# xguo7/SND-VAE

Measured on AMD Instinct MI355X. Metric: training graphs/sec + ELBO-step ms, N=4096 d=64, at 1/2/4/8 MI355X, higher is better.
Workload: dtype bf16; 1 GPU; C2: node-latent SND-VAE train step, N=4096, d=64, 8 graphs/GPU, HIP-graph replay; n_nodes=4096, latent=64, graphs_per_gpu=8, global_batch=8, parallelism=dp1, hip_graph=True

## Files before the change

### snd_vae_amd/csrc/snd_common.hpp

```cpp
#pragma once
#include <hip/hip_runtime.h>
#include <cstdint>
#include <cstdio>
#include <string>

#include "../../include/snd_vae.h"

namespace snd {

void set_error(const char* fmt, ...);

#define SND_CHECK_ARG(cond, ...)                                   \
  do {                                                             \
    if (!(cond)) {                                                 \
      ::snd::set_error(__VA_ARGS__);                               \
      return SND_ERR_ARG;                                          \
    }                                                              \
  } while (0)

#define SND_LAUNCH_CHECK(what)                                     \
  do {                                                             \
    hipError_t e_ = hipGetLastError();                             \
    if (e_ != hipSuccess) {                                        \
      ::snd::set_error("%s: %s", what, hipGetErrorString(e_));     \
      return SND_ERR_HIP;                                          \
    }                                                              \
  } while (0)

#define SND_TRY(expr)                                              \
  do {                                                             \
    int rc_ = (expr);                                              \
    if (rc_ != 0) return rc_;                                      \
  } while (0)

constexpr float kBnC = 0.99950037468777325f;
constexpr float kLeak = 0.2f;
constexpr float kLog2e = 1.4426950408889634f;
constexpr float kLn2 = 0.69314718055994531f;
constexpr double kSoftplusM1 = 0.31326168751822286;

#ifndef SND_MEAS
#define SND_MEAS 0
#endif
constexpr int kKeepDbg = 1 << 23;
__host__ __device__ __forceinline__ constexpr int kdbg(int dbg) { return SND_MEAS ? dbg : (dbg & kKeepDbg); }

__device__ __forceinline__ float lrelu(float x) { return fmaxf(x, kLeak * x); }
__device__ __forceinline__ float lrelu_grad(float x) { return x >= 0.f ? 1.f : kLeak; }

inline int device_cu_count() {
  static const int n = [] {
    int d = 0, v = 0;
    if (hipGetDevice(&d) != hipSuccess ||
        hipDeviceGetAttribute(&v, hipDeviceAttributeMultiprocessorCount, d) != hipSuccess || v <= 0) {
      (void)hipGetLastError();
      return 256;
    }
    return v;
  }();
  return n;
}

__device__ __forceinline__ void edge_ce_terms(float x, float pw, float& coef, float& loss) {
  coef = -pw;
  if (pw != 1.f) {
    const float e = __expf(-fabsf(x));
    const float q = 1.f + e;
    const float r = __builtin_amdgcn_rcpf(q);
    const float sg = x >= 0.f ? r : e * r;
    coef += (pw - 1.f) * sg;
    loss += (pw - 1.f) * (fmaxf(x, 0.f) + __logf(q));
  }
}

__device__ __forceinline__ float kl_elem(float s, float mu) {
  const float x = 2.f * s;
  float r;
// ... 113 lines not shown
```

### snd_vae_amd/csrc/snd_dec.hip

```cpp
#include "snd_dec.hpp"

#include <algorithm>

namespace snd {
namespace {

constexpr int DT = 1024;
constexpr int NW = DT / 64;
constexpr int kDynLds = 148 * 1024;

typedef __attribute__((address_space(1))) const void* gptr_t;
typedef __attribute__((address_space(3))) void* lptr_t;

__device__ __forceinline__ void dglds16(const void* g, void* lds_base) {
  __builtin_amdgcn_global_load_lds((gptr_t)g, (lptr_t)lds_base, 16, 0, 0);
}
__host__ __device__ __forceinline__ int dswz(int row, int kp) {
  return kp == 128 ? (row & 15) : (kp == 64 ? ((row >> 1) & 7) : 0);
}
__host__ __device__ __forceinline__ int lkc_of(int kp) { return kp == 128 ? 4 : (kp == 64 ? 3 : 2); }
__host__ __device__ __forceinline__ int img_bytes(int rows, int kp) {
  return ((rows * kp * 2) + 1023) & ~1023;
}
__host__ __device__ __forceinline__ int rup(int a, int b) { return (a + b - 1) / b * b; }
// ... 21 lines not shown
    ldY2n = rup(max(p.m2.b, 1), 4);
    w = 0; a = wb; b = a + max(ja, ua); c = b + max(u1, u3);
    total = c + TR * ldY2n * 4;
  }
};
struct BwdLay {
  int w, d3, d2, d1, cps, total, tapb;
  __host__ __device__ BwdLay(const DecChainBwdArgs& p, int TR, bool str = false) {
    tapb = max(max(tap_bytes(p.k3t), tap_bytes(p.k2t)), tap_bytes(p.k1t));
    const int wb = str ? 2 * tapb : max(max(p.k3t.np * p.k3t.kp, p.k2t.np * p.k2t.kp), p.k1t.np * p.k1t.kp) * 5 * 2;
    const int nw = NW;
    w = 0;
    d3 = wb;
    d2 = d3 + img_bytes(in_rows(TR + 8), p.k3t.kp);
    d1 = d2 + img_bytes(in_rows(TR + 4), p.k2t.kp);
    cps = d1 + img_bytes(in_rows(TR), p.k1t.kp);
    const int c1 = (nw / ((p.k2t.np / 16 + 1) / 2)) * 3 * p.k2t.np;
    const int c2 = (nw / (p.k3t.np / 16)) * 3 * p.k3t.np;
    total = cps + max(c1, c2) * 4;
  }
};

struct Tile { int r0, rend, glo, ghi; };
template <int TR>
__device__ __forceinline__ Tile tile_of(int t, int npg) {
  const int tpg = (npg + TR - 1) / TR;
  const int g = t / tpg, lt = t - g * tpg;
  Tile x;
  x.glo = g * npg; x.ghi = x.glo + npg;
  x.r0 = x.glo + lt * TR; x.rend = min(x.r0 + TR, x.ghi);
  return x;
}

template <int NWV = NW>
__device__ __forceinline__ void stage_window(const __bf16* src, int ld, int K, int wr0, int nrows,
                                             int nvalid, int glo, int ghi, int kp, char* img,
                                             const void* zero) {
  const int lane = threadIdx.x & 63, w = threadIdx.x >> 6;
  const int lk = lkc_of(kp), kc = 1 << lk;
  const int npc = ((nrows << lk) + 63) >> 6;
  for (int j = w; j < npc; j += NWV) {
    const int q = (j << 6) + lane;
    const int row = q >> lk, pc = q & (kc - 1);
    const int c = pc ^ dswz(row, kp);
    const int gr = wr0 + row;
    const bool v = row < nvalid && gr >= glo && gr < ghi && 8 * c < K;
    const void* g = v ? (const void*)(src + (long long)gr * ld + 8 * c) : zero;
    dglds16(g, img + (j << 10));
  }
}
__device__ __forceinline__ void stage_weights(const DecImg& im, char* dst, int dbg) {
  if (dbg & 1) return;
  const int lane = threadIdx.x & 63, w = threadIdx.x >> 6;
  const int npc = (5 * im.np * im.kp * 2) >> 10;
  const char* g = reinterpret_cast<const char*>(im.w) + lane * 16;
  for (int j = w; j < npc; j += NW) dglds16(g + (j << 10), dst + (j << 10));
}
__device__ __forceinline__ void dglds16_async(const void* g, void* lds_base) {
  const unsigned dst = __builtin_amdgcn_readfirstlane((unsigned)(uintptr_t)(lptr_t)lds_base);
  unsigned keep;
  asm volatile("s_mov_b32 %0, m0\n\ts_mov_b32 m0, %2\n\ts_nop 0\n\t"
               "global_load_lds_dwordx4 %1, off\n\ts_mov_b32 m0, %0"
               : "=&s"(keep) : "v"(g), "s"(dst) : "memory");
}
__device__ __forceinline__ void stage_weights_async(const DecImg& im, char* dst, int dbg) {
  if (dbg & 1) return;
  const int lane = threadIdx.x & 63, w = threadIdx.x >> 6;
  const int npc = (5 * im.np * im.kp * 2) >> 10;
  const char* g = reinterpret_cast<const char*>(im.w) + lane * 16;
  for (int j = w; j < npc; j += NW) dglds16_async(g + (j << 10), dst + (j << 10));
}
template <int NWV>
__device__ __forceinline__ void stage_tap_async(const DecImg& im, int t, char* dst, int dbg) {
  if (dbg & 1) return;
  const int lane = threadIdx.x & 63, w = threadIdx.x >> 6;
  const int npc = tap_bytes(im) >> 10;
  const char* g = reinterpret_cast<const char*>(im.w) + (long long)t * tap_bytes(im) + lane * 16;
  for (int j = w; j < npc; j += NWV) dglds16_async(g + (j << 10), dst + (j << 10));
}
__host__ __device__ __forceinline__ int wimg_bytes(const DecImg& im) { return 5 * im.np * im.kp * 2; }
__device__ __forceinline__ void wait_dma() {
  __builtin_amdgcn_s_waitcnt(0x0F70);
  __syncthreads();
}

__device__ __forceinline__ __bf16* img_at(__bf16* img, int row, int kp, int n0) {
  return img + row * kp + ((((n0 >> 3) ^ dswz(row, kp)) << 3) | (n0 & 4));
}

template <int NBH, int KCS, class Pre, class Epi>
__device__ __forceinline__ void conv_phase_t(const __bf16* xs, int kpx, const __bf16* ws, int kpw, int np,
                                             int n_out, Pre&& pre, Epi&& epi, int dbg) {
  const int lane = threadIdx.x & 63, w = __builtin_amdgcn_readfirstlane(threadIdx.x >> 6);
  const int li = lane & 15, lg = lane >> 4;
  const int nrb = (n_out + 15) >> 4, nbc = np >> 4;
  const int ncg = (nbc + NBH - 1) / NBH, wpc = NW / ncg;
// ... 93 lines not shown
        const __bf16* xrp = xs + xrow * kpx;
        const int xsw = dswz(xrow, kpx);
        auto chunk = [&](int ks) {
          const int ch = 4 * ks + lg;
          const bf16x8 bx = *reinterpret_cast<const bf16x8*>(xrp + ((ch ^ xsw) << 3));
#pragma unroll
          for (int i = 0; i < NBH; ++i) {
            const bf16x8 aw = *reinterpret_cast<const bf16x8*>(wrp + wb[i] + ((ch ^ wsw) << 3));
            acc[j][i] = __builtin_amdgcn_mfma_f32_16x16x32_bf16(aw, bx, acc[j][i], 0, 0, 0);
          }
        };
        if (KCS > 0 && kpw == 32 * KCS) {
#pragma unroll
          for (int ks = 0; ks < KCS; ++ks) chunk(ks);
        } else {
          for (int ks = 0; ks < (kpw >> 5); ++ks) chunk(ks);
        }
      }
    }
  }
  if (!act) return;
#pragma unroll
  for (int j = 0; j < MAXRB; ++j) {
    const int rb = k0 + j * wpc;
    if (rb >= nrb) break;
    epi(16 * rb + li, nb0, acc[j], yp[j]);
  }
}

__device__ __forceinline__ float colpar(const ColMap& m, int n, const float* A, const float* Bv) {
  if (!m.valid(n) || !A) return 0.f;
  if (n < m.a || !Bv) return A[n < m.a ? n : m.logical(n)];
  return Bv[n - m.offb];
}

template <int CIN, int COUT, int SCR>
__device__ __forceinline__ void head_tile(int hi, int orow, bool rv, long long gr, const float (&u)[CIN],
                                          const float (&yv)[CIN], const float* hp, const float (&tg)[COUT],
                                          float count, float* yhat, __bf16* dyp, float* scr,
                                          double* sscr) {
  float wv[CIN][COUT], bv[COUT], gk[CIN], bk[CIN];
#pragma unroll
  for (int k = 0; k < CIN; ++k) {
#pragma unroll
    for (int o = 0; o < COUT; ++o) wv[k][o] = hp[k * COUT + o];
    gk[k] = hp[24 + k] * kBnC;
    bk[k] = hp[24 + CIN + k];
  }
#pragma unroll
  for (int o = 0; o < COUT; ++o) bv[o] = hp[20 + o];
  float dp[COUT];
  double sse = 0.0;
#pragma unroll
  for (int o = 0; o < COUT; ++o) {
    float zo = bv[o];
#pragma unroll
    for (int k = 0; k < CIN; ++k) zo += u[k] * wv[k][o];
    const float yh = 1.f / (1.f + __expf(-zo));
    const float diff = yh - tg[o];
    if (rv) {
      if (yhat) yhat[gr * COUT + o] = yh;
      sse += (double)diff * diff;
    }
    dp[o] = rv ? 2.f * diff / count * yh * (1.f - yh) : 0.f;
  }
  float dt[CIN], dyv[CIN];
// ... 49 lines not shown
  __bf16* u2img = jimg;
  __bf16* u1img = reinterpret_cast<__bf16*>(smem + L.b);
  float* u3 = reinterpret_cast<float*>(smem + L.b);
  float* y3 = u3 + TR * 16;
  float* y2n = reinterpret_cast<float*>(smem + L.c);
  const int kpu2 = a.m2.phys() <= 32 ? 32 : (a.m2.phys() <= 64 ? 64 : 128);
  const int own = tl.rend - tl.r0;
  const bool stamp = kdbg(a.dbg) & (1 << 21);
  unsigned long long ts[9] = {};
  if (stamp) ts[0] = __builtin_amdgcn_s_memrealtime();

  if (kdbg(a.dbg) & (1 << 23)) {
    for (int i = tid * 16; i < L.total - L.a; i += DTK * 16)
      *reinterpret_cast<uint4*>(smem + L.a + i) = make_uint4(~0u, ~0u, ~0u, ~0u);
    __syncthreads();
  }
  if (!(kdbg(a.dbg) & 32)) {
    const int kpo = a.k2.kp, npc = (kpo - a.k1.np) >> 2, nr = in_rows(TR + 4);
    for (int i = tid; i < nr * 4; i += DTK) {
      const int row = i >> 2, q = i & 3;
      if (q < npc) *reinterpret_cast<bf16x4*>(img_at(u1img, row, kpo, a.k1.np + 4 * q)) = bf16x4{};
    }
  }
  __syncthreads();
  if (!(kdbg(a.dbg) & 16))
    stage_window<NWV>(a.zb, a.ldz, a.dj, tl.r0 - 6, in_rows(TR + 8), own + 12, tl.glo, tl.ghi, a.k1.kp,
                      reinterpret_cast<char*>(jimg), a.zero);
  char* tb0 = reinterpret_cast<char*>(wimg);
  char* tb1 = tb0 + L.tapb;
  if constexpr (STR) stage_tap_async<NWV>(a.k1, 0, tb0, kdbg(a.dbg));
  else stage_weights(a.k1, reinterpret_cast<char*>(wimg), kdbg(a.dbg));
  constexpr int HPT = DTK == 1024 ? 512 : DTK - 128;
  static_assert(DTK - 128 >= 2 * TR || DTK == 1024, "dec_fwd: head parameter threads overlap the targets'");
  if (tid >= HPT && tid < HPT + 128) {
    const int i = tid - HPT, hh = i >> 6, j = i & 63;
    const int cin = hh ? 20 : 10, cout = hh ? 1 : 2;
    const float* w = hh ? a.wn : a.ws;
    const float* b = hh ? a.bn : a.bs;
    const float* g = hh ? a.g2n : a.g3;
    const float* be = hh ? a.be2n : a.be3;
    float v = 0.f;
    if (j < cin * cout) v = w[j];
    else if (j >= 20 && j < 20 + cout) v = b[j - 20];
    else if (j >= 24 && j < 24 + cin) v = g[j - 24];
    else if (j >= 24 + cin && j < 24 + 2 * cin) v = be[j - 24 - cin];
    hp[hh][j] = v;
  }
  float tg[2] = {0.f, 0.f};
  if (tid < 2 * TR) {
    const int orow = tid % TR;
    const long long gr = tl.r0 + orow;
    if (orow < own) {
      if (tid < TR) { tg[0] = a.s_truth[gr * 2]; tg[1] = a.s_truth[gr * 2 + 1]; }
      else tg[0] = a.x_truth[gr];
    }
  }
  if (tid < 128) {
    const int n = tid;
    cp1[0][n] = colpar(a.m1, n, a.b1, nullptr);
    cp1[1][n] = colpar(a.m1, n, a.g1, nullptr) * kBnC;
    cp1[2][n] = colpar(a.m1, n, a.be1, nullptr);
    cp2[0][n] = colpar(a.m2, n, a.b2s, a.b2n);
    cp2[1][n] = colpar(a.m2, n, a.g2s, a.g2n) * kBnC;
    cp2[2][n] = colpar(a.m2, n, a.be2s, a.be2n);
    if (n < 16) {
      const ColMap m3{a.s3, 0, a.s3};
      cp3[0][n] = colpar(m3, n, a.b3, nullptr);
      cp3[1][n] = colpar(m3, n, a.g3, nullptr) * kBnC;
      cp3[2][n] = colpar(m3, n, a.be3, nullptr);
    }
  }
  wait_dma();
  if (stamp) ts[1] = __builtin_amdgcn_s_memrealtime();

  auto nopre = [](int, int, auto&) {};
  {
    const int wr0 = tl.r0 - 4, n_out = own + 8, kpo = a.k2.kp, nbc = a.k1.np >> 4;
    auto epi1 = [&](int orow, int nb0, f32x4 (&acc)[2], f32x4 (&)[2]) {
      if (orow >= n_out) return;
      const int gr = wr0 + orow;
      const bool ing = gr >= tl.glo && gr < tl.ghi, mine = gr >= tl.r0 && gr < tl.rend;
#pragma unroll
      for (int i = 0; i < 2; ++i) {
        if (nb0 + i >= nbc) continue;
        const int n0 = 16 * (nb0 + i) + 4 * lg;
        const f32x4 b = *reinterpret_cast<const f32x4*>(&cp1[0][n0]);
        const f32x4 g = *reinterpret_cast<const f32x4*>(&cp1[1][n0]);
        const f32x4 be = *reinterpret_cast<const f32x4*>(&cp1[2][n0]);
        f32x4 yv;
        bf16x4 ub;
#pragma unroll
        for (int e = 0; e < 4; ++e) {
          yv[e] = acc[i][e] + b[e];
          ub[e] = (__bf16)(ing ? lrelu(yv[e] * g[e] + be[e]) : 0.f);
        }
        *reinterpret_cast<bf16x4*>(img_at(u1img, orow, kpo, n0)) = ub;
        if (mine && !(kdbg(a.dbg) & 8)) {
          *reinterpret_cast<f32x4*>(a.y1 + (long long)gr * a.ldy1 + n0) = yv;
          *reinterpret_cast<bf16x4*>(a.u1 + (long long)gr * a.ldy1 + n0) = ub;
        }
      }
    };
// ... 97 lines not shown
        }
        const float t1[1] = {tg[0]};
        head_tile<20, 1, SCR>(1, orow, rv, gr, u, yv, hp[1], t1, a.cnt_n, a.xhat, a.dy2 + gr * a.lddy2 + a.m2.offb,
                              scr + NQS * SCR, sscr + TR);
      }
    }
    __syncthreads();
    if (stamp) ts[7] = __builtin_amdgcn_s_memrealtime();
    if (tid < NQS + NQN) {
      const float* src = scr + tid * SCR;
      float v = 0.f;
#pragma unroll 32
      for (int r = 0; r < TR; ++r) v += src[r];
      if (tid < NQS) a.phs[(long long)t * NQS + tid] = v;
      else a.phn[(long long)t * NQN + tid - NQS] = v;
    } else if (tid >= 256 && tid < 258) {
      const double* src = sscr + TR * (tid - 256);
      double v = 0.0;
#pragma unroll 32
      for (int r = 0; r < TR; ++r) v += src[r];
      (tid == 256 ? a.sse_s : a.sse_n)[t] = v;
    }
  }
  if (stamp) {
    __syncthreads();
    if (tid == 0) {
      ts[8] = __builtin_amdgcn_s_memrealtime();
      unsigned* o = reinterpret_cast<unsigned*>(a.phs + (long long)t * NQS);
      for (int k = 0; k < 9; ++k) o[k] = (unsigned)ts[k];
    }
  }
}

template <int NBH>
__device__ __forceinline__ void colpart_flush(float (&q)[3][NBH][4], float* slots, int np, int nb0, int nbc,
                                              int slot) {
  const int lane = threadIdx.x & 63, li = lane & 15, lg = lane >> 4;
#pragma unroll
  for (int k = 0; k < 3; ++k)
#pragma unroll
    for (int i = 0; i < NBH; ++i)
#pragma unroll
      for (int e = 0; e < 4; ++e) {
        const float v = row16_sum(q[k][i][e]);
        const int n = 16 * (nb0 + i) + 4 * lg + e;
        if (li == 0 && nb0 + i < nbc) slots[(slot * 3 + k) * np + n] = v;
      }
}

template <int TR, int NWV = NW, bool STR = false>
__global__ void __launch_bounds__(64 * NWV) __attribute__((amdgpu_waves_per_eu(4, 4)))
dec_bwd_kernel(DecChainBwdArgs a) {
  constexpr int DTK = 64 * NWV;
  extern __shared__ __attribute__((aligned(16))) char smem[];
  __shared__ __attribute__((aligned(16))) float cpa[2][128], cpb[2][128];
  const BwdLay L(a, TR, STR);
  const Tile tl = tile_of<TR>(blockIdx.x, a.npg);
  const int tid = threadIdx.x, w = tid >> 6, lane = tid & 63, lg = lane >> 4;
  __bf16* wimg = reinterpret_cast<__bf16*>(smem + L.w);
  __bf16* d3 = reinterpret_cast<__bf16*>(smem + L.d3);
  __bf16* d2 = reinterpret_cast<__bf16*>(smem + L.d2);
  __bf16* d1 = reinterpret_cast<__bf16*>(smem + L.d1);
  float* slots = reinterpret_cast<float*>(smem + L.cps);
  const int own = tl.rend - tl.r0;
  const int t = blockIdx.x;
  const bool stamp = kdbg(a.dbg) & (1 << 21);
  unsigned long long ts[8] = {};
  if (stamp) ts[0] = __builtin_amdgcn_s_memrealtime();

  if (!(kdbg(a.dbg) & 32))
    for (int i = tid * 16; i < L.cps - L.d3; i += DTK * 16)
      *reinterpret_cast<uint4*>(smem + L.d3 + i) = make_uint4(0u, 0u, 0u, 0u);
  __syncthreads();
  if (!(kdbg(a.dbg) & 16))
    stage_window<NWV>(a.dy3, a.lddy3, a.s3, tl.r0 - 6, in_rows(TR + 8), own + 12, tl.glo, tl.ghi, a.k3t.kp,
                      reinterpret_cast<char*>(d3), a.zero);
  const int wb3 = L.d3 - L.w, k3o = wb3 - wimg_bytes(a.k3t);
  const bool pre2 = !STR && wimg_bytes(a.k2t) <= k3o && (k3o & 1023) == 0;
  __bf16* wimg3 = pre2 ? wimg + k3o / 2 : wimg;
  char* tb0 = reinterpret_cast<char*>(wimg);
  char* tb1 = tb0 + L.tapb;
  if constexpr (STR) stage_tap_async<NWV>(a.k3t, 0, tb0, kdbg(a.dbg));
  else stage_weights(a.k3t, reinterpret_cast<char*>(wimg3), kdbg(a.dbg));
  if (tid < 128) {
    const int n = tid;
    const ColMap ms{a.m2.a, 0, a.m2.a};
    cpa[0][n] = colpar(ms, n, a.g2s, nullptr) * kBnC;
    cpa[1][n] = colpar(ms, n, a.be2s, nullptr);
    cpb[0][n] = colpar(a.m1, n, a.g1, nullptr) * kBnC;
    cpb[1][n] = colpar(a.m1, n, a.be1, nullptr);
  }
  {
    const int wr0 = tl.r0 - 4, nv = own + 8, kp2 = a.k2t.kp;
    const int nq = (a.m2.b + 3) / 4;
    for (int i = tid; i < ((kdbg(a.dbg) & 16) ? 0 : nv * nq); i += DTK) {
      const int row = i / nq, q = i - row * nq;
      const int gr = wr0 + row;
      if (gr < tl.glo || gr >= tl.ghi) continue;
      const int n0 = a.m2.offb + 4 * q;
      const bf16x4 v = *reinterpret_cast<const bf16x4*>(a.dy2 + (long long)gr * a.lddy2 + n0);
      *reinterpret_cast<bf16x4*>(img_at(d2, row, kp2, n0)) = v;
    }
  }
  wait_dma();
  if (!STR && pre2) stage_weights_async(a.k2t, reinterpret_cast<char*>(wimg), kdbg(a.dbg));
  if (stamp) ts[1] = __builtin_amdgcn_s_memrealtime();
  {
    const int wr0 = tl.r0 - 4, n_out = own + 8, N = a.m2.a, kpo = a.k2t.kp;
    const int nbc = a.k3t.np >> 4, ncg = nbc, wpc = NWV / ncg;
    const int nb0 = w % ncg;
    float q[3][1][4] = {};
    auto pre3t = [&](int orow, int nb, f32x4 (&yp)[1]) {
                    yp[0] = f32x4{0.f, 0.f, 0.f, 0.f};
                    const int gr = wr0 + orow;
                    if (orow < n_out && gr >= tl.glo && gr < tl.ghi) {
                      const int n0 = 16 * nb + 4 * lg;
                      const float* p = a.y2 + (long long)gr * a.ldy2 + n0;
#pragma unroll
                      for (int e = 0; e < 4; ++e) if (n0 + e < N) yp[0][e] = p[e];
                    }
                  };
    auto epi3t = [&](int orow, int nb, f32x4 (&acc)[1], f32x4 (&yp)[1]) {
      if (orow >= n_out) return;
      const int gr = wr0 + orow;
      const bool ing = gr >= tl.glo && gr < tl.ghi, mine = gr >= tl.r0 && gr < tl.rend;
      const int n0 = 16 * nb + 4 * lg;
      const f32x4 ga = *reinterpret_cast<const f32x4*>(&cpa[0][n0]);
      const f32x4 be = *reinterpret_cast<const f32x4*>(&cpa[1][n0]);
      float o[4];
#pragma unroll
      for (int e = 0; e < 4; ++e) {
        const float dt = ing ? acc[0][e] * lrelu_grad(yp[0][e] * ga[e] + be[e]) : 0.f;
        o[e] = dt * ga[e];
        if (mine) { q[0][0][e] += dt * yp[0][e]; q[1][0][e] += dt; q[2][0][e] += o[e]; }
      }
      bf16x4 ob;
#pragma unroll
      for (int e = 0; e < 4; ++e) ob[e] = (__bf16)o[e];
      if (n0 < a.m2.offb || !a.m2.b)
        *reinterpret_cast<bf16x4*>(img_at(d2, orow, kpo, n0)) = ob;
      if (mine && !(kdbg(a.dbg) & 8)) {
        __bf16* dp = a.dy2 + (long long)gr * a.lddy2 + n0;
        if (n0 + 3 < N) *reinterpret_cast<bf16x4*>(dp) = ob;
        else
#pragma unroll
          for (int e = 0; e < 4; ++e) if (n0 + e < N) dp[e] = ob[e];
      }
    };
    if constexpr (STR)
      conv_phase_str<1, 1, NWV, 2>(d3, a.k3t.kp, a.k3t, tb0, tb1, 0, &a.k2t, n_out, pre3t, epi3t, a.dbg);
    else conv_phase<1, 1>(d3, a.k3t.kp, wimg3, a.k3t.kp, a.k3t.np, n_out, pre3t, epi3t, a.dbg);
    if (w / ncg < wpc) colpart_flush<1>(q, slots, a.k3t.np, nb0, nbc, w / ncg);
    __syncthreads();
    for (int i = tid; i < 3 * N; i += DTK) {
      const int k = i / N, n = i - k * N;
      float s = 0.f;
      for (int sl = 0; sl < wpc; ++sl) s += slots[(sl * 3 + k) * a.k3t.np + n];
      a.pc2s[(long long)t * 3 * N + i] = s;
    }
  }
  __syncthreads();
  if (stamp) ts[2] = __builtin_amdgcn_s_memrealtime();
  if constexpr (!STR) {
    if (!pre2) stage_weights(a.k2t, reinterpret_cast<char*>(wimg), kdbg(a.dbg));
    wait_dma();
  }
  if (stamp) ts[3] = __builtin_amdgcn_s_memrealtime();
  {
    const int wr0 = tl.r0 - 2, n_out = own + 4, W1 = a.m1.phys(), kpo = a.k1t.kp;
    const int nbc = a.k2t.np >> 4, ncg = (nbc + 1) / 2, wpc = NWV / ncg;
    const int nb0 = 2 * (w % ncg);
    float q[3][2][4] = {};
    auto pre2t = [&](int orow, int nb, f32x4 (&yp)[2]) {
                    const int gr = wr0 + orow;
                    const bool ok = orow < n_out && gr >= tl.glo && gr < tl.ghi;
#pragma unroll
                    for (int i = 0; i < 2; ++i) {
                      yp[i] = f32x4{0.f, 0.f, 0.f, 0.f};
                      const int n0 = 16 * (nb + i) + 4 * lg;
                      if (ok && nb + i < nbc) yp[i] = *reinterpret_cast<const f32x4*>(a.y1 + (long long)gr * a.ldy1 + n0);
                    }
                  };
    auto epi2t = [&](int orow, int nb, f32x4 (&acc)[2], f32x4 (&yp)[2]) {
      if (orow >= n_out) return;
      const int gr = wr0 + orow;
      const bool ing = gr >= tl.glo && gr < tl.ghi, mine = gr >= tl.r0 && gr < tl.rend;
#pragma unroll
      for (int i = 0; i < 2; ++i) {
        if (nb + i >= nbc) continue;
        const int n0 = 16 * (nb + i) + 4 * lg;
        const f32x4 ga = *reinterpret_cast<const f32x4*>(&cpb[0][n0]);
        const f32x4 be = *reinterpret_cast<const f32x4*>(&cpb[1][n0]);
        float o[4];
#pragma unroll
        for (int e = 0; e < 4; ++e) {
          const float dt = ing ? acc[i][e] * lrelu_grad(yp[i][e] * ga[e] + be[e]) : 0.f;
          o[e] = dt * ga[e];
          if (mine) { q[0][i][e] += dt * yp[i][e]; q[1][i][e] += dt; q[2][i][e] += o[e]; }
        }
        bf16x4 ob;
#pragma unroll
        for (int e = 0; e < 4; ++e) ob[e] = (__bf16)o[e];
        *reinterpret_cast<bf16x4*>(img_at(d1, orow, kpo, n0)) = ob;
        if (mine && !(kdbg(a.dbg) & 8)) *reinterpret_cast<bf16x4*>(a.dy1 + (long long)gr * a.lddy1 + n0) = ob;
      }
    };
    if constexpr (STR)
      conv_phase_str<2, 2, NWV, 3>(d2, a.k2t.kp, a.k2t, tb0, tb1, 5, &a.k1t, n_out, pre2t, epi2t, a.dbg);
    else conv_phase<2, 2>(d2, a.k2t.kp, wimg, a.k2t.kp, a.k2t.np, n_out, pre2t, epi2t, a.dbg);
    __syncthreads();
    if (w / ncg < wpc) colpart_flush<2>(q, slots, a.k2t.np, nb0, nbc, w / ncg);
    __syncthreads();
    for (int i = tid; i < 3 * W1; i += DTK) {
      const int k = i / W1, n = i - k * W1;
      float s = 0.f;
      for (int sl = 0; sl < wpc; ++sl) s += slots[(sl * 3 + k) * a.k2t.np + n];
      a.pc1[(long long)t * 3 * W1 + i] = s;
    }
  }
  __syncthreads();
  if (stamp) ts[4] = __builtin_amdgcn_s_memrealtime();
  if constexpr (!STR) {
    stage_weights(a.k1t, reinterpret_cast<char*>(wimg), kdbg(a.dbg));
    wait_dma();
  }
  if (stamp) ts[5] = __builtin_amdgcn_s_memrealtime();
  {
    const int n_out = own, N = a.dj;
    auto nopre = [](int, int, auto&) {};
    auto epi1t = [&](int orow, int nb, f32x4 (&acc)[2], f32x4 (&)[2]) {
      if (orow >= n_out) return;
// ... 135 lines not shown
```

### snd_vae_amd/csrc/snd_fast.hip

```cpp
#include "snd_fast.hpp"
#include "snd_gather.hpp"
#include "snd_pack.hpp"

#include <algorithm>

namespace snd {

namespace {

constexpr int NT = 256;

typedef short v4s __attribute__((ext_vector_type(4)));
typedef short v8s __attribute__((ext_vector_type(8)));
typedef __attribute__((address_space(3))) v4s lds_v4s;

__device__ __forceinline__ int swz(int row, int kp) {
  return kp >= 128 ? (row & 15) : (kp == 64 ? ((row >> 1) & 7) : 0);
}

__device__ __forceinline__ uint4 pack8(float4 lo, float4 hi) {
  bf16x8 v;
  v[0] = (__bf16)lo.x; v[1] = (__bf16)lo.y; v[2] = (__bf16)lo.z; v[3] = (__bf16)lo.w;
  v[4] = (__bf16)hi.x; v[5] = (__bf16)hi.y; v[6] = (__bf16)hi.z; v[7] = (__bf16)hi.w;
  return __builtin_bit_cast(uint4, v);
// ... 548 lines not shown
    }
  }
  if (kdbg(a.dbg) & 8) return;
  const int sK = a.sK, sn4 = a.sn4;
#pragma unroll
  for (int i = 0; i < NPW; ++i) {
    const int k = 16 * cbs[i] + li;
    if (!pvs[i] || k >= a.K) continue;
    float* row = a.slab + (long long)bx * T * sK * sn4 + ((long long)ts[i] * sK + a.wk0 + k) * sn4 + a.wn0;
#pragma unroll
    for (int ob = 0; ob < NBO; ++ob) {
      const int n0 = 16 * ob + 4 * lg;
      if (n0 < a.N)
        *reinterpret_cast<float4*>(row + n0) =
            make_float4(acc[i][ob][0], acc[i][ob][1], acc[i][ob][2], acc[i][ob][3]);
    }
  }
}

template <int NBO>
__global__ void __launch_bounds__(WGT) wgrad_kernel(WgArgs a) {
  extern __shared__ __attribute__((aligned(16))) __bf16 lds[];
  wgrad_body<NBO>(a, blockIdx.x, blockIdx.y, lds);
}

struct WgMultiPack {
  WgArgs a[kMaxWgMulti];
  int start[kMaxWgMulti + 1];
  int nseg;
  int stamp_base;
};
static_assert(sizeof(WgMultiPack) <= 4096, "wgrad_multi: kernel arguments over 4 KB");

__global__ void __launch_bounds__(WGT) __attribute__((amdgpu_waves_per_eu(8, 8)))
wgrad_multi_kernel(WgMultiPack m) {
  extern __shared__ __attribute__((aligned(16))) __bf16 lds[];
  __shared__ unsigned tsl[kWgStampWords];
  const bool stamp = (kdbg(m.a[0].dbg) & (1 << 21)) && m.a[0].stamps;
  wg_stamp(tsl, 0, stamp);
  if (kdbg(m.a[0].dbg) & 1) return;
  const int bid = blockIdx.y * gridDim.x + blockIdx.x;
  int s = 0;
  if (gridDim.y > 1) {
    s = blockIdx.y;
  } else {
#pragma unroll
    for (int i = 1; i < kMaxWgMulti; ++i) s += (int)blockIdx.x >= m.start[i] ? 1 : 0;
  }
  s = __builtin_amdgcn_readfirstlane(s);
  const WgArgs a = m.a[s];
  const int local = gridDim.y > 1 ? (int)blockIdx.x : (int)blockIdx.x - m.start[s];
  const int gx = cdiv_d(a.R, a.rows_per_wg);
  const int bx = local % gx, by = local / gx;
  const bool two = a.pairs_per_wg > WGT / 64;
  if (kdbg(a.dbg) & 16) return;
  unsigned* ts = stamp ? tsl : nullptr;
  wg_stamp(ts, 1, stamp);
  switch ((a.N + 15) >> 4) {
    case 1: if (two) wgrad_body<1, 2>(a, bx, by, lds, ts); else wgrad_body<1>(a, bx, by, lds, ts); break;
    case 2: if (two) wgrad_body<2, 2>(a, bx, by, lds, ts); else wgrad_body<2>(a, bx, by, lds, ts); break;
    case 3: if (two) wgrad_body<3, 2>(a, bx, by, lds, ts); else wgrad_body<3>(a, bx, by, lds, ts); break;
    default: if (two) wgrad_body<4, 2>(a, bx, by, lds, ts); else wgrad_body<4>(a, bx, by, lds, ts); break;
  }
  if (stamp) {
    __syncthreads();
    if (threadIdx.x == 0) {
      unsigned* o = m.a[0].stamps + ((long long)m.stamp_base + bid) * kWgStampWords;
      for (int i = 0; i < 9; ++i) o[i] = tsl[i];
      o[9] = (unsigned)__builtin_amdgcn_s_memrealtime();
      o[10] = __builtin_amdgcn_s_getreg((31 << 11) | 4);
      o[11] = __builtin_amdgcn_s_getreg((31 << 11) | 20);
    }
  }
}

struct HeadFastPack { HeadFastArgs h[2]; };

template <int CIN, int COUT>
__device__ __forceinline__ void head_rows(const HeadFastArgs& h, int R) {
  constexpr int NQ = CIN * COUT + COUT + 3 * CIN;
  __shared__ float red[16][NQ];
  __shared__ double sred[4];
  const int tid = threadIdx.x, lane = tid & 63, w = tid >> 6;
  const int r = blockIdx.x * kHeadFastRows + tid;
// ... 255 lines not shown
}

static WgArgs wg_norm(const WgArgs& a) {
  WgArgs x = a;
  if (x.sK == 0) { x.sK = x.K; x.sn4 = wgrad_n4(x.N); x.wk0 = 0; x.wn0 = 0; }
  return x;
}

#ifndef SND_WG_SPLIT_LDS
#define SND_WG_SPLIT_LDS (80 * 1024)
#endif
constexpr size_t kWgSplitLds = SND_WG_SPLIT_LDS;
static int wg_split(const WgArgs& a, WgArgs* out, int cap) {
  const bool sk = a.K > 64 && wg_lds_bytes(a.T, a.K, std::min(a.N, 64)) > kWgSplitLds, sn = a.N > 64;
  int n = 0;
  for (int k0 = 0; k0 < a.K; k0 += sk ? 64 : a.K)
    for (int n0 = 0; n0 < a.N; n0 += sn ? 64 : a.N) {
      if (n >= cap) return -1;
      WgArgs w = a;
      w.K = sk ? std::min(64, a.K - k0) : a.K;
      w.N = sn ? std::min(64, a.N - n0) : a.N;
      w.x = static_cast<const __bf16*>(a.x) + k0;
      w.dy = static_cast<const __bf16*>(a.dy) + n0;
      w.wk0 = a.wk0 + k0; w.wn0 = a.wn0 + n0;
      w.pairs_per_wg = std::min(a.pairs_per_wg, a.T * cdiv(w.K, 16));
      out[n++] = w;
    }
  return n;
}

static int wg_multi_flush(WgMultiPack& pk, int total, size_t lds, hipStream_t s) {
  if (pk.nseg == 0) return 0;
  for (int i = pk.nseg; i <= kMaxWgMulti; ++i) pk.start[i] = total;
  bool uniform = pk.nseg > 1;
  for (int i = 1; i < pk.nseg; ++i) uniform = uniform && pk.start[i + 1] - pk.start[i] == pk.start[1];
  const dim3 grid = uniform ? dim3(pk.start[1], pk.nseg) : dim3(total);
  hipLaunchKernelGGL(wgrad_multi_kernel, grid, dim3(WGT), lds, s, pk);
  SND_LAUNCH_CHECK("wgrad_multi_kernel");
  return 0;
}

int launch_wgrad_multi(const WgArgs* a, int n, hipStream_t s) {
  if (n <= 0) return 0;
  WgMultiPack pk{};
  size_t lds = 0;
  int total = 0, base = 0;
  pk.nseg = 0;
  const bool stamps = a[0].stamps != nullptr;
  for (int i = 0; i < n; ++i) {
    const WgArgs x0 = wg_norm(a[i]);
    if (x0.R <= 0) continue;
    SND_CHECK_ARG(x0.T == 1 || x0.T == 5, "wgrad_multi: T must be 1 or 5");
    SND_CHECK_ARG(x0.K > 0 && x0.K <= 128 && x0.N > 0 && x0.N <= 128, "wgrad_multi: K %d N %d", x0.K, x0.N);
    SND_CHECK_ARG(x0.ldx % 8 == 0 && x0.lddy % 8 == 0 && x0.x_bf16 && x0.dy_bf16,
                  "wgrad_multi: bf16 operands with leading dims %% 8");
    SND_CHECK_ARG(x0.rows_per_wg % kRcRows == 0 && x0.pairs_per_wg >= 1 && x0.pairs_per_wg <= 2 * WGT / 64,
                  "wgrad_multi: geometry");
    SND_CHECK_ARG(x0.x && x0.dy && x0.slab && x0.zero && x0.npg > 0, "wgrad_multi: null operand");
    SND_CHECK_ARG(x0.sn4 % 4 == 0 && x0.wn0 % 4 == 0 && x0.wk0 + x0.K <= x0.sK &&
                  x0.wn0 + wgrad_n4(x0.N) <= x0.sn4, "wgrad_multi: slab window");
    WgArgs win[4];
    const int nw = wg_split(x0, win, 4);
    SND_CHECK_ARG(nw > 0, "wgrad_multi: window split");
    for (int j = 0; j < nw; ++j) {
      if (pk.nseg == kMaxWgMulti) {
        SND_TRY(wg_multi_flush(pk, total, lds, s));
        base += total;
// ... 102 lines not shown
```

Baseline: 38850 graphs/s.

## Issue decoder prologue loads asynchronously and pin wgrad multi-segment args in SGPRs

Result: no change. 39180 graphs/s, median of 6 (+0.8%).

```diff
diff --git a/snd_vae_amd/csrc/snd_common.hpp b/snd_vae_amd/csrc/snd_common.hpp
--- a/snd_vae_amd/csrc/snd_common.hpp
+++ b/snd_vae_amd/csrc/snd_common.hpp
@@ -42,7 +42,7 @@
 #ifndef SND_MEAS
 #define SND_MEAS 0
 #endif
-constexpr int kKeepDbg = 1 << 23;
+constexpr int kKeepDbg = (1 << 23) | (1 << 24);
 __host__ __device__ __forceinline__ constexpr int kdbg(int dbg) { return SND_MEAS ? dbg : (dbg & kKeepDbg); }
 
 __device__ __forceinline__ float lrelu(float x) { return fmaxf(x, kLeak * x); }
diff --git a/snd_vae_amd/csrc/snd_dec.hip b/snd_vae_amd/csrc/snd_dec.hip
--- a/snd_vae_amd/csrc/snd_dec.hip
+++ b/snd_vae_amd/csrc/snd_dec.hip
@@ -77,7 +77,14 @@
   return x;
 }
 
-template <int NWV = NW>
+__device__ __forceinline__ void dglds16_async(const void* g, void* lds_base) {
+  const unsigned dst = __builtin_amdgcn_readfirstlane((unsigned)(uintptr_t)(lptr_t)lds_base);
+  unsigned keep;
+  asm volatile("s_mov_b32 %0, m0\n\ts_mov_b32 m0, %2\n\ts_nop 0\n\t"
+               "global_load_lds_dwordx4 %1, off\n\ts_mov_b32 m0, %0"
+               : "=&s"(keep) : "v"(g), "s"(dst) : "memory");
+}
+template <int NWV = NW, bool ASYNC = false>
 __device__ __forceinline__ void stage_window(const __bf16* src, int ld, int K, int wr0, int nrows,
                                              int nvalid, int glo, int ghi, int kp, char* img,
                                              const void* zero) {
@@ -91,7 +98,8 @@
     const int gr = wr0 + row;
     const bool v = row < nvalid && gr >= glo && gr < ghi && 8 * c < K;
     const void* g = v ? (const void*)(src + (long long)gr * ld + 8 * c) : zero;
-    dglds16(g, img + (j << 10));
+    if constexpr (ASYNC) dglds16_async(g, img + (j << 10));
+    else dglds16(g, img + (j << 10));
   }
 }
 __device__ __forceinline__ void stage_weights(const DecImg& im, char* dst, int dbg) {
@@ -100,13 +108,6 @@
   const int npc = (5 * im.np * im.kp * 2) >> 10;
   const char* g = reinterpret_cast<const char*>(im.w) + lane * 16;
   for (int j = w; j < npc; j += NW) dglds16(g + (j << 10), dst + (j << 10));
-}
-__device__ __forceinline__ void dglds16_async(const void* g, void* lds_base) {
-  const unsigned dst = __builtin_amdgcn_readfirstlane((unsigned)(uintptr_t)(lptr_t)lds_base);
-  unsigned keep;
-  asm volatile("s_mov_b32 %0, m0\n\ts_mov_b32 m0, %2\n\ts_nop 0\n\t"
-               "global_load_lds_dwordx4 %1, off\n\ts_mov_b32 m0, %0"
-               : "=&s"(keep) : "v"(g), "s"(dst) : "memory");
 }
 __device__ __forceinline__ void stage_weights_async(const DecImg& im, char* dst, int dbg) {
   if (dbg & 1) return;
@@ -266,6 +267,13 @@
   if (!m.valid(n) || !A) return 0.f;
   if (n < m.a || !Bv) return A[n < m.a ? n : m.logical(n)];
   return Bv[n - m.offb];
+}
+
+__device__ __forceinline__ const float* colpar_ptr(const ColMap& m, int n, const float* A, const float* Bv,
+                                                   const float* zero) {
+  if (!m.valid(n) || !A) return zero;
+  if (n < m.a || !Bv) return A + (n < m.a ? n : m.logical(n));
+  return Bv + (n - m.offb);
 }
 
 template <int CIN, int COUT, int SCR>
@@ -381,42 +389,57 @@
   else stage_weights(a.k1, reinterpret_cast<char*>(wimg), kdbg(a.dbg));
   constexpr int HPT = DTK == 1024 ? 512 : DTK - 128;
   static_assert(DTK - 128 >= 2 * TR || DTK == 1024, "dec_fwd: head parameter threads overlap the targets'");
-  if (tid >= HPT && tid < HPT + 128) {
-    const int i = tid - HPT, hh = i >> 6, j = i & 63;
+  const float* zf = reinterpret_cast<const float*>(a.zero);
+  const ColMap m3{a.s3, 0, a.s3};
+  const float* pp[12];
+  {
+    const int n = tid;
+    pp[0] = colpar_ptr(a.m1, n, a.b1, nullptr, zf);
+    pp[1] = colpar_ptr(a.m1, n, a.g1, nullptr, zf);
+    pp[2] = colpar_ptr(a.m1, n, a.be1, nullptr, zf);
+    pp[3] = colpar_ptr(a.m2, n, a.b2s, a.b2n, zf);
+    pp[4] = colpar_ptr(a.m2, n, a.g2s, a.g2n, zf);
+    pp[5] = colpar_ptr(a.m2, n, a.be2s, a.be2n, zf);
+    pp[6] = colpar_ptr(m3, n, a.b3, nullptr, zf);
+    pp[7] = colpar_ptr(m3, n, a.g3, nullptr, zf);
+    pp[8] = colpar_ptr(m3, n, a.be3, nullptr, zf);
+    const int i = tid - HPT, hh = (i >> 6) & 1, j = i & 63;
     const int cin = hh ? 20 : 10, cout = hh ? 1 : 2;
     const float* w = hh ? a.wn : a.ws;
     const float* b = hh ? a.bn : a.bs;
     const float* g = hh ? a.g2n : a.g3;
     const float* be = hh ? a.be2n : a.be3;
-    float v = 0.f;
-    if (j < cin * cout) v = w[j];
-    else if (j >= 20 && j < 20 + cout) v = b[j - 20];
-    else if (j >= 24 && j < 24 + cin) v = g[j - 24];
-    else if (j >= 24 + cin && j < 24 + 2 * cin) v = be[j - 24 - cin];
-    hp[hh][j] = v;
-  }
-  float tg[2] = {0.f, 0.f};
-  if (tid < 2 * TR) {
+    const float* ph = zf;
+    if (j < cin * cout) ph = w + j;
+    else if (j >= 20 && j < 20 + cout) ph = b + (j - 20);
+    else if (j >= 24 && j < 24 + cin) ph = g + (j - 24);
+    else if (j >= 24 + cin && j < 24 + 2 * cin) ph = be + (j - 24 - cin);
+    pp[9] = (tid >= HPT && tid < HPT + 128) ? ph : zf;
     const int orow = tid % TR;
     const long long gr = tl.r0 + orow;
-    if (orow < own) {
-      if (tid < TR) { tg[0] = a.s_truth[gr * 2]; tg[1] = a.s_truth[gr * 2 + 1]; }
-      else tg[0] = a.x_truth[gr];
-    }
-  }
+    const bool tv = tid < 2 * TR && orow < own;
+    pp[10] = !tv ? zf : (tid < TR ? a.s_truth + gr * 2 : a.x_truth + gr);
+    pp[11] = tv && tid < TR ? a.s_truth + gr * 2 + 1 : zf;
+  }
+  float pv[12];
+#pragma unroll
+  for (int k = 0; k < 12; ++k) pv[k] = *pp[k];
+#pragma unroll
+  for (int k = 0; k < 12; ++k) asm volatile("" : "+v"(pv[k]));
+  if (tid >= HPT && tid < HPT + 128) hp[(tid - HPT) >> 6][(tid - HPT) & 63] = pv[9];
+  const float tg[2] = {pv[10], pv[11]};
   if (tid < 128) {
     const int n = tid;
-    cp1[0][n] = colpar(a.m1, n, a.b1, nullptr);
-    cp1[1][n] = colpar(a.m1, n, a.g1, nullptr) * kBnC;
-    cp1[2][n] = colpar(a.m1, n, a.be1, nullptr);
-    cp2[0][n] = colpar(a.m2, n, a.b2s, a.b2n);
-    cp2[1][n] = colpar(a.m2, n, a.g2s, a.g2n) * kBnC;
-    cp2[2][n] = colpar(a.m2, n, a.be2s, a.be2n);
+    cp1[0][n] = pv[0];
+    cp1[1][n] = pv[1] * kBnC;
+    cp1[2][n] = pv[2];
+    cp2[0][n] = pv[3];
+    cp2[1][n] = pv[4] * kBnC;
+    cp2[2][n] = pv[5];
     if (n < 16) {
-      const ColMap m3{a.s3, 0, a.s3};
-      cp3[0][n] = colpar(m3, n, a.b3, nullptr);
-      cp3[1][n] = colpar(m3, n, a.g3, nullptr) * kBnC;
-      cp3[2][n] = colpar(m3, n, a.be3, nullptr);
+      cp3[0][n] = pv[6];
+      cp3[1][n] = pv[7] * kBnC;
+      cp3[2][n] = pv[8];
     }
   }
   wait_dma();
@@ -580,6 +603,10 @@
   }
 }
 
+__device__ __forceinline__ float mul_then_add(float a, float b, float c) {
+#pragma clang fp contract(off)
+  return a * b + c;
+}
 template <int NBH>
 __device__ __forceinline__ void colpart_flush(float (&q)[3][NBH][4], float* slots, int np, int nb0, int nbc,
                                               int slot) {
@@ -616,29 +643,28 @@
   unsigned long long ts[8] = {};
   if (stamp) ts[0] = __builtin_amdgcn_s_memrealtime();
 
-  if (!(kdbg(a.dbg) & 32))
-    for (int i = tid * 16; i < L.cps - L.d3; i += DTK * 16)
-      *reinterpret_cast<uint4*>(smem + L.d3 + i) = make_uint4(0u, 0u, 0u, 0u);
-  __syncthreads();
-  if (!(kdbg(a.dbg) & 16))
-    stage_window<NWV>(a.dy3, a.lddy3, a.s3, tl.r0 - 6, in_rows(TR + 8), own + 12, tl.glo, tl.ghi, a.k3t.kp,
-                      reinterpret_cast<char*>(d3), a.zero);
   const int wb3 = L.d3 - L.w, k3o = wb3 - wimg_bytes(a.k3t);
   const bool pre2 = !STR && wimg_bytes(a.k2t) <= k3o && (k3o & 1023) == 0;
   __bf16* wimg3 = pre2 ? wimg + k3o / 2 : wimg;
   char* tb0 = reinterpret_cast<char*>(wimg);
   char* tb1 = tb0 + L.tapb;
-  if constexpr (STR) stage_tap_async<NWV>(a.k3t, 0, tb0, kdbg(a.dbg));
-  else stage_weights(a.k3t, reinterpret_cast<char*>(wimg3), kdbg(a.dbg));
-  if (tid < 128) {
-    const int n = tid;
-    const ColMap ms{a.m2.a, 0, a.m2.a};
-    cpa[0][n] = colpar(ms, n, a.g2s, nullptr) * kBnC;
-    cpa[1][n] = colpar(ms, n, a.be2s, nullptr);
-    cpb[0][n] = colpar(a.m1, n, a.g1, nullptr) * kBnC;
-    cpb[1][n] = colpar(a.m1, n, a.be1, nullptr);
-  }
-  {
+  if constexpr (STR) {
+    if (!(kdbg(a.dbg) & 32))
+      for (int i = tid * 16; i < L.cps - L.d3; i += DTK * 16)
+        *reinterpret_cast<uint4*>(smem + L.d3 + i) = make_uint4(0u, 0u, 0u, 0u);
+    __syncthreads();
+    if (!(kdbg(a.dbg) & 16))
+      stage_window<NWV>(a.dy3, a.lddy3, a.s3, tl.r0 - 6, in_rows(TR + 8), own + 12, tl.glo, tl.ghi, a.k3t.kp,
+                        reinterpret_cast<char*>(d3), a.zero);
+    stage_tap_async<NWV>(a.k3t, 0, tb0, kdbg(a.dbg));
+    if (tid < 128) {
+      const int n = tid;
+      const ColMap ms{a.m2.a, 0, a.m2.a};
+      cpa[0][n] = colpar(ms, n, a.g2s, nullptr) * kBnC;
+      cpa[1][n] = colpar(ms, n, a.be2s, nullptr);
+      cpb[0][n] = colpar(a.m1, n, a.g1, nullptr) * kBnC;
+      cpb[1][n] = colpar(a.m1, n, a.be1, nullptr);
+    }
     const int wr0 = tl.r0 - 4, nv = own + 8, kp2 = a.k2t.kp;
     const int nq = (a.m2.b + 3) / 4;
     for (int i = tid; i < ((kdbg(a.dbg) & 16) ? 0 : nv * nq); i += DTK) {
@@ -648,6 +674,53 @@
       const int n0 = a.m2.offb + 4 * q;
       const bf16x4 v = *reinterpret_cast<const bf16x4*>(a.dy2 + (long long)gr * a.lddy2 + n0);
       *reinterpret_cast<bf16x4*>(img_at(d2, row, kp2, n0)) = v;
+    }
+  } else {
+    if (kdbg(a.dbg) & (1 << 24)) {
+      for (int i = tid * 16; i < L.cps - L.d3; i += DTK * 16)
+        *reinterpret_cast<uint4*>(smem + L.d3 + i) = make_uint4(~0u, ~0u, ~0u, ~0u);
+      __syncthreads();
+    }
+    if (!(kdbg(a.dbg) & 16))
+      stage_window<NWV, true>(a.dy3, a.lddy3, a.s3, tl.r0 - 6, in_rows(TR + 8), own + 12, tl.glo, tl.ghi,
+                              a.k3t.kp, reinterpret_cast<char*>(d3), a.zero);
+    stage_weights_async(a.k3t, reinterpret_cast<char*>(wimg3), kdbg(a.dbg));
+    const float* zf = reinterpret_cast<const float*>(a.zero);
+    const int wr0n = tl.r0 - 4, kp2 = a.k2t.kp;
+    const int nq = (a.m2.b + 3) / 4;
+    const int nit = (kdbg(a.dbg) & 16) ? 0 : (own + 8) * nq;
+    auto dy2_item = [&](int i, int& row, int& n0) -> const uint2* {
+      row = i / max(nq, 1);
+      n0 = a.m2.offb + 4 * (i - row * nq);
+      const int gr = wr0n + row;
+      const bool v = i < nit && gr >= tl.glo && gr < tl.ghi;
+      return reinterpret_cast<const uint2*>(v ? (const void*)(a.dy2 + (long long)gr * a.lddy2 + n0) : a.zero);
+    };
+    const ColMap ms{a.m2.a, 0, a.m2.a};
+    int row0, n00;
+    const uint2* dp0 = dy2_item(tid, row0, n00);
+    float pv[4] = {*colpar_ptr(ms, tid, a.g2s, nullptr, zf), *colpar_ptr(ms, tid, a.be2s, nullptr, zf),
+                   *colpar_ptr(a.m1, tid, a.g1, nullptr, zf), *colpar_ptr(a.m1, tid, a.be1, nullptr, zf)};
+    uint2 dv0 = *dp0;
+    if (!(kdbg(a.dbg) & 32))
+      for (int i = tid * 16; i < L.cps - L.d2; i += DTK * 16)
+        *reinterpret_cast<uint4*>(smem + L.d2 + i) = make_uint4(0u, 0u, 0u, 0u);
+    __syncthreads();
+#pragma unroll
+    for (int k = 0; k < 4; ++k) asm volatile("" : "+v"(pv[k]));
+    asm volatile("" : "+v"(dv0.x), "+v"(dv0.y));
+    if (tid < 128) {
+      const int n = tid;
+      cpa[0][n] = pv[0] * kBnC;
+      cpa[1][n] = pv[1];
+      cpb[0][n] = pv[2] * kBnC;
+      cpb[1][n] = pv[3];
+    }
+    if (tid < nit) *reinterpret_cast<uint2*>(img_at(d2, row0, kp2, n00)) = dv0;
+    for (int i = tid + DTK; i < nit; i += DTK) {
+      int row, n0;
+      const uint2 v = *dy2_item(i, row, n0);
+      *reinterpret_cast<uint2*>(img_at(d2, row, kp2, n0)) = v;
     }
   }
   wait_dma();
@@ -680,7 +753,12 @@
       for (int e = 0; e < 4; ++e) {
         const float dt = ing ? acc[0][e] * lrelu_grad(yp[0][e] * ga[e] + be[e]) : 0.f;
         o[e] = dt * ga[e];
-        if (mine) { q[0][0][e] += dt * yp[0][e]; q[1][0][e] += dt; q[2][0][e] += o[e]; }
+        if (mine) {
+          if constexpr (STR) q[0][0][e] += dt * yp[0][e];
+          else q[0][0][e] = __builtin_fmaf(dt, yp[0][e], q[0][0][e]);
+          q[1][0][e] += dt;
+          q[2][0][e] += o[e];
+        }
       }
       bf16x4 ob;
 #pragma unroll
@@ -744,7 +822,13 @@
         for (int e = 0; e < 4; ++e) {
           const float dt = ing ? acc[i][e] * lrelu_grad(yp[i][e] * ga[e] + be[e]) : 0.f;
           o[e] = dt * ga[e];
-          if (mine) { q[0][i][e] += dt * yp[i][e]; q[1][i][e] += dt; q[2][i][e] += o[e]; }
+          if (mine) {
+            const bool fused = i == 0 ? (e == 1 || e == 2) : e < 2;
+            if constexpr (STR) q[0][i][e] += dt * yp[i][e];
+            else q[0][i][e] = fused ? __builtin_fmaf(dt, yp[i][e], q[0][i][e]) : mul_then_add(dt, yp[i][e], q[0][i][e]);
+            q[1][i][e] += dt;
+            q[2][i][e] += o[e];
+          }
         }
         bf16x4 ob;
 #pragma unroll
diff --git a/snd_vae_amd/csrc/snd_fast.hip b/snd_vae_amd/csrc/snd_fast.hip
--- a/snd_vae_amd/csrc/snd_fast.hip
+++ b/snd_vae_amd/csrc/snd_fast.hip
@@ -604,6 +604,12 @@
 };
 static_assert(sizeof(WgMultiPack) <= 4096, "wgrad_multi: kernel arguments over 4 KB");
 
+__device__ __forceinline__ void wg_pin(WgArgs& a) {
+  asm volatile("" : "+s"(a.x), "+s"(a.ldx), "+s"(a.K), "+s"(a.dy), "+s"(a.lddy), "+s"(a.N), "+s"(a.R),
+               "+s"(a.npg), "+s"(a.T), "+s"(a.rows_per_wg), "+s"(a.pairs_per_wg), "+s"(a.slab), "+s"(a.zero),
+               "+s"(a.dbg), "+s"(a.sK), "+s"(a.sn4), "+s"(a.wk0), "+s"(a.wn0));
+}
+
 __global__ void __launch_bounds__(WGT) __attribute__((amdgpu_waves_per_eu(8, 8)))
 wgrad_multi_kernel(WgMultiPack m) {
   extern __shared__ __attribute__((aligned(16))) __bf16 lds[];
@@ -612,16 +618,30 @@
   wg_stamp(tsl, 0, stamp);
   if (kdbg(m.a[0].dbg) & 1) return;
   const int bid = blockIdx.y * gridDim.x + blockIdx.x;
-  int s = 0;
-  if (gridDim.y > 1) {
-    s = blockIdx.y;
-  } else {
-#pragma unroll
-    for (int i = 1; i < kMaxWgMulti; ++i) s += (int)blockIdx.x >= m.start[i] ? 1 : 0;
-  }
-  s = __builtin_amdgcn_readfirstlane(s);
-  const WgArgs a = m.a[s];
-  const int local = gridDim.y > 1 ? (int)blockIdx.x : (int)blockIdx.x - m.start[s];
+  int gy = gridDim.y;
+  WgArgs a = m.a[blockIdx.y];
+  int st[kMaxWgMulti];
+#pragma unroll
+  for (int i = 1; i < kMaxWgMulti; ++i) st[i] = m.start[i];
+  asm volatile("" : "+s"(gy));
+#pragma unroll
+  for (int i = 1; i < kMaxWgMulti; ++i) asm volatile("" : "+s"(st[i]));
+  wg_pin(a);
+  int local = blockIdx.x;
+  if (gy <= 1) {
+    int s = 0, s0 = 0;
+#pragma unroll
+    for (int i = 1; i < kMaxWgMulti; ++i) {
+      const bool in = (int)blockIdx.x >= st[i];
+      s += in ? 1 : 0;
+      s0 = in ? max(s0, st[i]) : s0;
+    }
+    local = (int)blockIdx.x - s0;
+    if (s) {
+      a = m.a[s];
+      wg_pin(a);
+    }
+  }
   const int gx = cdiv_d(a.R, a.rows_per_wg);
   const int bx = local % gx, by = local / gx;
   const bool two = a.pairs_per_wg > WGT / 64;
@@ -943,7 +963,7 @@
 static int wg_multi_flush(WgMultiPack& pk, int total, size_t lds, hipStream_t s) {
   if (pk.nseg == 0) return 0;
   for (int i = pk.nseg; i <= kMaxWgMulti; ++i) pk.start[i] = total;
-  bool uniform = pk.nseg > 1;
+  bool uniform = pk.nseg > 1 && !(debug_flags() & (1 << 26));
   for (int i = 1; i < pk.nseg; ++i) uniform = uniform && pk.start[i + 1] - pk.start[i] == pk.start[1];
   const dim3 grid = uniform ? dim3(pk.start[1], pk.nseg) : dim3(total);
   hipLaunchKernelGGL(wgrad_multi_kernel, grid, dim3(WGT), lds, s, pk);
```
